# endoli/fiksi

Measured on AMD Instinct MI355X. Metric: Gauss-Newton iters/sec + converged systems/sec, 100k×32-constraint f64 batch, higher is better.
Workload: dtype f64

## Files before the change

fiksi_amd/csrc/fx_grouped.hip:

```cpp
#include <hip/hip_runtime.h>
#include <stdint.h>
#include <algorithm>
#include <cstdio>
#include <cstdlib>
#include <utility>

#include "fx_device.h"
#include "fx_expr.h"
#include "fx_grouped_rows.h"
#include "fx_wave.h"

#ifndef FX_GROUPED_LADDER
#define FX_GROUPED_LADDER 1
#endif

namespace fx {

struct GroupLayout {
    uint32_t vt, mr;
    uint32_t off_xs, off_a, off_rhs, off_g, off_r, off_p, off_gvar, off_rtag, off_vout, off_pw, off_pe;
    uint32_t off_colof, off_gcol, off_fidx;
    uint32_t pw_cap, pe_cap;
    uint32_t stride;
    uint32_t tab_bytes, off_qx;
// ... 626 lines not shown
                            const int tag = (int)(b.expr_tag[e0 + i] & 0x7F);
                            const ushort4 f4 = reinterpret_cast<const ushort4*>(b.expr_idx)[e0 + i];
                            uint16_t ff[4] = {f4.x, f4.y, f4.z, f4.w};
                            uint32_t vars8[8] = {0, 0, 0, 0, 0, 0, 0, 0};
                            const int k = expand_vars(tag, ff, vars8);
                            double prm_e = b.expr_param[e0 + i];
                            if ((prm.mode & 1u) && (tag == FX_TAG_PPD || tag == FX_TAG_PLD)) prm_e = scale_recip * prm_e;
                            rtag[pos] = (uint8_t)tag;
                            P[pos] = (T)prm_e;
#pragma unroll
                            for (int e = 0; e < 8; ++e) {
                                gvar[pos * 8 + e] = (uint16_t)vars8[e];
                                gcol[pos * 8 + e] = (e < k) ? (int8_t)colof[vars8[e]] : (int8_t)-1;
                            }
                        }
                    }
                }
                if (!UNITS && !reuse) {
                    nfree = 0;
                    bool any_var = false;
                    for_vars([&](uint32_t i, double v, uint32_t info) {
                        const bool member = i < nvt && (info & VAR_COMP_MASK) == c;
                        const bool in = member && !(info & VAR_FIXED_BIT);
                        const uint32_t m = gballot(in);
                        const uint32_t pos = nfree + (uint32_t)__popc(m & below);
                        if (i < nvt) colof[i] = in ? (int16_t)pos : (int16_t)-1;
                        if (in && pos < (uint32_t)N) fidx[pos] = (uint16_t)i;
                        if (i < (uint32_t)(RS * PF)) {
                            const int cc = in ? (int)pos : -1;
                            if (i < (uint32_t)RS) c_col[0] = cc; else if (i < 2u * RS) c_col[1] = cc; else c_col[2] = cc;
                        }
                        if (in && (prm.mode & 2u)) {
                            uint32_t st = lcg_jump(rng, 2u * pos);
                            st = st * 1664525u + 1013904223u;
                            const double f1 = (1.0 / 4294967295.0) * (double)st;
                            st = st * 1664525u + 1013904223u;
                            const double f2 = (1.0 / 4294967295.0) * (double)st;
                            double x = (prm.mode & 1u) ? v * scale_recip : v;
                            x += x * (1.0 / 8196.0) * f1 + (1.0 / 65568.0) * f2;
                            XS[i] = (T)x;
                        }
                        nfree += (uint32_t)__popc(m);
                        any_var = any_var || gballot(member) != 0u;
                    });
                    if (!any_var) {
                        c += 1;
                    } else {
                        have_comp = true;
                        rows_listed = true;
                        built = true;
                        built_cls = cls;
                        if (prm.mode & 2u) rng = lcg_jump(rng, 2u * nfree);
                        group_sync();
#pragma unroll
                        for (int q = 0; q < NC; ++q) {
                            const uint32_t j = (uint32_t)(hl + RS * q);
                            my_vi[q] = (j < nfree) ? (uint32_t)fidx[j] : 0u;
                        }
                        m_rows = 0;
                        for_exprs([&](uint32_t i, int tag, double prm_e, uint32_t comp, ushort4 f4) {
                            const bool in = (i < net) && (comp == c);
                            const uint32_t mk = gballot(in);
                            const uint32_t pos = m_rows + (uint32_t)__popc(mk & below);
                            if (i < (uint32_t)(RS * PF)) {
                                const int rr = in ? (int)pos : -1;
                                if (i < (uint32_t)RS) c_row[0] = rr; else if (i < 2u * RS) c_row[1] = rr; else c_row[2] = rr;
                            }
                            if (in) {
                                uint16_t ff[4] = {f4.x, f4.y, f4.z, f4.w};
                                uint32_t vars8[8] = {0, 0, 0, 0, 0, 0, 0, 0};
                                const int k = expand_vars(tag, ff, vars8);
                                if ((prm.mode & 1u) && (tag == FX_TAG_PPD || tag == FX_TAG_PLD)) prm_e = scale_recip * prm_e;
                                rtag[pos] = (uint8_t)tag;
                                P[pos] = (T)prm_e;
#pragma unroll
                                for (int e = 0; e < 8; ++e) {
                                    gvar[pos * 8 + e] = (uint16_t)vars8[e];
                                    gcol[pos * 8 + e] = (e < k) ? (int8_t)colof[vars8[e]] : (int8_t)-1;
                                }
                            }
                            m_rows += (uint32_t)__popc(mk);
                        });
                    }
                }
                if (rows_listed) {
                    group_sync();
#pragma unroll
                    for (int q = 0; q < NC; ++q) {
                        xstart[q] = ((uint32_t)(hl + RS * q) < nfree) ? XS[my_vi[q]] : T(0);
                        xc[q] = xstart[q];
                    }
                    n_pw = 0;
                    n_pe = 0;
                    for (uint32_t at = 0; !QRG && at < m_rows; at += RS) {
                        const uint32_t row = at + (uint32_t)hl;
                        uint32_t mask = 0;
                        uint64_t cols = 0;
                        if (row < m_rows) {
#pragma unroll
                            for (int e = 0; e < 8; ++e) {
                                const int cc = gcol[row * 8 + e];
                                mask |= (cc >= 0) ? (1u << e) : 0u;
                                cols |= (uint64_t)(uint8_t)cc << (8 * e);
                            }
                        }
                        const uint32_t kf = (uint32_t)__popc(mask);
                        uint32_t np = kf * (kf + 1u) / 2u;
                        for (uint32_t m1 = mask; m1; m1 &= m1 - 1u) {
                            const uint32_t a = (uint32_t)__ffs(m1) - 1u;
                            for (uint32_t m2 = m1 & (m1 - 1u); m2; m2 &= m2 - 1u) {
                                const uint32_t bb = (uint32_t)__ffs(m2) - 1u;
                                np += (((cols >> (8u * a)) ^ (cols >> (8u * bb))) & 0xFFu) == 0u;
                            }
                        }
                        uint32_t inc2 = np, inc1 = kf;
#pragma unroll
                        for (int off = 1; off < RS; off <<= 1) {
                            const uint32_t t2 = (uint32_t)__shfl_up((int)inc2, off, RS), t1 = (uint32_t)__shfl_up((int)inc1, off, RS);
                            if (hl >= off) {
                                inc2 += t2;
                                inc1 += t1;
                            }
                        }
                        uint32_t at2 = n_pw + inc2 - np, at1 = n_pe + inc1 - kf;
                        if (at2 + np <= L.pw_cap && at1 + kf <= L.pe_cap) {
                            for (uint32_t m1 = mask; m1; m1 &= m1 - 1u) {
                                const uint32_t a = (uint32_t)__ffs(m1) - 1u;
                                const uint32_t ca = (uint32_t)(cols >> (8u * a)) & 0xFFu;
                                PE[at1++] = (uint16_t)((row << (3 + CB)) | (a << CB) | ca);
                                for (uint32_t m2 = m1; m2; m2 &= m2 - 1u) {
                                    const uint32_t bb = (uint32_t)__ffs(m2) - 1u;
                                    const uint32_t cb = (uint32_t)(cols >> (8u * bb)) & 0xFFu;
                                    const uint32_t hi = ca > cb ? ca : cb, lo = ca > cb ? cb : ca;
                                    const uint32_t w = (row << 19) | (a << 16) | (bb << 13) | tri_at(hi, lo);
                                    PW[at2++] = w;
                                    if (a != bb && ca == cb) PW[at2++] = w;
                                }
                            }
                        }
                        n_pw += (uint32_t)__shfl((int)inc2, RS - 1, RS);
                        n_pe += (uint32_t)__shfl((int)inc1, RS - 1, RS);
                    }
                    group_sync();
                    if constexpr (PWR > 0) {
#pragma unroll
                        for (int u = 0; u < PWR; ++u) {
                            const uint32_t t = (uint32_t)(u * RS + hl);
                            pw_reg[u] = (t < n_pw && t < L.pw_cap) ? PW[t] : 0xFFFFFFFFu;
                        }
#pragma unroll
                        for (int u = 0; u < PER; ++u) {
                            const uint32_t t = (uint32_t)(u * RS + hl);
                            pe_reg[u] = (t < n_pe && t < L.pe_cap) ? (uint32_t)PE[t] : 0xFFFFFFFFu;
                        }
                    }
                }
                if (have_comp) {
                    stamp(GH_SETUP);
                    lambda = o.lambda0;
                    accepted = 0;
                    trials = 0;
                    outer = 0;
                    exit_code = FX_EXIT_MAX_OUTER;
                    fresh = true;
                    phase = GP_RUN;
                    if (n_pw > L.pw_cap || n_pe > L.pe_cap) {
                        sse = sse_start = T(0);
                        exit_code = FX_EXIT_NAN;
                        phase = GP_FINISH;
                    }
                }
            }
        }

        if constexpr (LADDER) {
            if (prm.ladder) {
                const unsigned long long bcand = __ballot(phase == GP_RUN && !fresh && lad_rank == 0);
                const unsigned long long bidle = __ballot(phase == GP_EXIT);
                if (bcand != 0ull && bidle != 0ull) {
                    uint32_t wid = 0, mem = 0, newlead = 0xFFFFu, newrank = 0;
#pragma unroll
                    for (int r = 0; r < 4; ++r) {
                        wid |= ((uint32_t)__builtin_amdgcn_readlane(lad_width, RS * r) & 15u) << (4 * r);
                        mem |= ((uint32_t)__builtin_amdgcn_readlane((int)lad_members, RS * r) & 255u) << (8 * r);
                    }
                    bool anyjoin = false;
#pragma unroll
                    for (int r = 0; r < 4; ++r) {
                        if (!((bidle >> (RS * r)) & 1ull)) continue;
                        uint32_t best = 15u, bw = 4u;
#pragma unroll
                        for (int l = 0; l < 4; ++l) {
                            const uint32_t w = (wid >> (4 * l)) & 15u;
                            if (((bcand >> (RS * l)) & 1ull) && w < bw) {
                                best = (uint32_t)l;
                                bw = w;
                            }
                        }
                        if (best != 15u) {
                            newlead = (newlead & ~(15u << (4 * r))) | (best << (4 * r));
                            newrank |= bw << (4 * r);
                            const uint32_t at = 8u * best + 2u * bw;
                            mem = (mem & ~(3u << at)) | ((uint32_t)r << at);
                            wid += 1u << (4u * best);
                            anyjoin = true;
                        }
                    }
                    if (anyjoin) {
                        const uint32_t nl = (newlead >> (4 * myrow)) & 15u;
                        const bool joining = nl != 15u;
                        const int grp = joining ? (int)nl : lad_lead;
                        const int srcl = grp * RS + hl;
                        auto cp = [&](auto& v) {
                            const auto t = lane_get(v, srcl);
                            if (joining) v = t;
                        };
                        cp(nfree); cp(m_rows); cp(n_pw); cp(n_pe); cp(trials); cp(accepted); cp(outer); cp(exit_code);
                        cp(sse); cp(lambda);
#pragma unroll
                        for (int q = 0; q < NC; ++q) {
                            cp(my_vi[q]); cp(xc[q]); cp(diag[q]); cp(rhs_l[q]);
                        }
                        if constexpr (PWR > 0) {
#pragma unroll
                            for (int u = 0; u < PWR; ++u) cp(pw_reg[u]);
#pragma unroll
                            for (int u = 0; u < PER; ++u) cp(pe_reg[u]);
                        }
                        lad_width = (int)((wid >> (4 * grp)) & 15u);
                        lad_members = (mem >> (8 * grp)) & 255u;
                        if (joining) {
                            lad_lead = (int)nl;
                            lad_rank = (int)((newrank >> (4 * myrow)) & 15u);
                            built = false;
                            using V = typename Vec16<T>::type;
                            const V* lb = reinterpret_cast<const V*>(rows0 + (uint32_t)nl * L.stride);
                            V* mine = reinterpret_cast<V*>(base);
                            for (uint32_t i = hl; i < L.stride / 16u; i += RS) mine[i] = lb[i];
                            fresh = false;
                            phase = GP_RUN;
                        }
                        group_sync();
                    }
                }
            }
        }

        int kmax;
        {
            const int km = (phase == GP_RUN && !fresh) ? (int)nfree : 0;
            const int k0 = __builtin_amdgcn_readlane(km, 0), k1 = __builtin_amdgcn_readlane(km, 16);
            const int k2 = __builtin_amdgcn_readlane(km, 32), k3 = __builtin_amdgcn_readlane(km, 48);
            kmax = max(max(k0, k1), max(k2, k3));
        }
        if (phase == GP_RUN) {
            stamp(GH_TAIL);
            int code = LC_FRESH;
            bool go = true;
            T delta[NC];
#pragma unroll
            for (int q = 0; q < NC; ++q) delta[q] = T(0);
            if (!fresh) {
                code = LC_REJECT;
                double lam_k = lambda;
                if constexpr (LADDER) {
                    if (lad_rank > 0)
                        for (int k = 0; k < lad_rank; ++k) lam_k *= o.reject_factor;
                }
                if (trials + (uint32_t)lad_rank >= o.max_trials) {
                    code = LC_CAP;
                    go = false;
                }
                if constexpr (QRG) {
                    if (go && !qr_step(lam_k, delta)) {
                        code = LC_SINGULAR;
                        go = false;
                    }
                }
                if (!QRG && go) {
                    int hv = hl;
                    asm volatile("" : "+v"(hv));
#pragma unroll
                    for (int q = 0; q < NC; ++q) At[tri_at((uint32_t)(hv + RS * q), (uint32_t)(hv + RS * q))] = diag[q] + (T)lam_k;
                    group_sync();
                    T a[NC][N];
#pragma unroll
                    for (int q = 0; q < NC; ++q) {
                        const int j = hv + RS * q;
                        const T* own = At + (uint32_t)(j * (j + 1) / 2);
                        const T* col = At + (uint32_t)j;
#pragma unroll
                        for (int i = 0; i < N; ++i) {
                            const int ti = i * (i + 1) / 2;
                            if (i <= RS * q) a[q][i] = own[i];
                            else if (i >= RS * (q + 1)) a[q][i] = col[ti];
                            else a[q][i] = ((hv >= i - RS * q) ? own : col + (ti - i))[i];
                        }
                    }
                    T invd[NC];
#pragma unroll
                    for (int q = 0; q < NC; ++q) invd[q] = T(1);
                    bool bad = false;
                    T acc[NC];
                    RBlock<NC, T, 0, UNITS>::template factor<false>(a, invd, acc, bad, hl, kmax);
                    stamp(GH_FACTOR);
                    if (bad) {
                        code = LC_SINGULAR;
                        go = false;
                    } else {
                        T invd2[NC];
#pragma unroll
                        for (int q = 0; q < NC; ++q) {
                            acc[q] = rhs_l[q];
                            invd2[q] = invd[q] * invd[q];
                        }
                        RBlock<NC, T, 0, UNITS>::forward(a, invd, acc, hl, kmax);
                        RBlock<NC, T, N / 8 - 1, UNITS>::backward(a, invd2, acc, hl, kmax);
#pragma unroll
                        for (int q = 0; q < NC; ++q) delta[q] = ((uint32_t)(hl + RS * q) < nfree) ? acc[q] * invd2[q] : T(0);
                    }
                }
                if (go) {
                    T dn2;
                    if constexpr (QRG) {
                        double acc = 0.0;
#pragma unroll
                        for (int q = 0; q < NC; ++q)
                            if ((uint32_t)(RS * q) < nfree) seq_add(acc, (double)delta[q] * (double)delta[q]);
                        dn2 = (T)acc;
                    } else {
                        dn2 = row_sum(delta[0] * delta[0]);
                        if constexpr (NC >= 2) dn2 = dn2 + row_sum(delta[1] * delta[1]);
                        if constexpr (NC >= 3) dn2 = dn2 + row_sum(delta[2] * delta[2]);
                    }
                    if (!(dn2 == dn2)) {
                        code = LC_NAN;
                        go = false;
                    } else if (dn2 < (T)o.step_tol) {
                        code = LC_STEP;
                        go = false;
                    }
                    stamp(GH_SOLVE);
                }
                if (go) {
#pragma unroll
                    for (int q = 0; q < NC; ++q)
                        if ((uint32_t)(hl + RS * q) < nfree) XS[my_vi[q]] = xc[q] + delta[q];
                    group_sync();
                }
            }
            T sse_t = T(0);
            if (go) {
                if constexpr (QRG) {
                    if (fresh) sse_t = eval_rows(std::true_type{});
                    else sse_t = eval_rows(std::false_type{});
                } else {
                    sse_t = eval_rows(std::true_type{});
                }
                stamp(GH_EVAL);
                if (!fresh) {
                    if (sse_t < sse) {
                        code = LC_ACCEPT;
                    } else {
                        double lam_k = lambda * o.reject_factor;
                        if constexpr (LADDER) {
                            if (lad_rank > 0)
                                for (int k = 0; k < lad_rank; ++k) lam_k *= o.reject_factor;
                        }
                        if (!(sse_t == sse_t) && !(lam_k < 1.0e300)) {
                            code = LC_REJ_NAN;
                        } else if (sizeof(T) == 4 && sse_t - sse <= (T)o.ftol * sse) {
                            code = LC_REJ_FTOL;
                        }
                    }
                }
            }
            int kw = (code != LC_REJECT) ? 0 : 1;
            int code_w = code;
            T sse_w = sse_t;
            T delta_w[NC];
#pragma unroll
            for (int q = 0; q < NC; ++q) delta_w[q] = delta[q];
            win_row = myrow;
            if constexpr (LADDER) {
                if (__ballot(lad_width > 1) != 0ull) {
                    int ck[4];
#pragma unroll
                    for (int k = 0; k < 4; ++k) ck[k] = lane_get(code, (int)((lad_members >> (2 * k)) & 3u) * RS + hl);
                    kw = lad_width;
                    code_w = LC_REJECT;
#pragma unroll
                    for (int k = 3; k >= 0; --k) {
                        if (k < lad_width && ck[k] != LC_REJECT) {
                            kw = k;
                            code_w = ck[k];
                        }
                    }
                    const int wrow = (int)((lad_members >> (2 * (kw < lad_width ? kw : 0))) & 3u);
                    const int wl = wrow * RS + hl;
                    sse_w = lane_get(sse_t, wl);
#pragma unroll
                    for (int q = 0; q < NC; ++q) delta_w[q] = lane_get(delta[q], wl);
                    win_row = wrow;
                }
            }
            bool assemble = false, fin = false;
            if (fresh) {
                sse = sse_t;
                sse_start = sse_t;
                assemble = true;
            } else {
                if (kw > 0) {
                    lambda *= o.reject_factor;
                    if constexpr (LADDER)
                        for (int k = 1; k < kw; ++k) lambda *= o.reject_factor;
                }
                if (kw == lad_width) {
                    trials += (uint32_t)kw;
                } else {
                    trials += (uint32_t)kw + (code_w != LC_CAP ? 1u : 0u);
                    if (code_w == LC_CAP) {
                        exit_code = FX_EXIT_TRIAL_CAP;
                        fin = true;
                    } else if (code_w == LC_SINGULAR) {
                        lambda *= o.singular_factor;
                    } else if (code_w == LC_NAN) {
                        exit_code = FX_EXIT_NAN;
                        fin = true;
                    } else if (code_w == LC_STEP) {
                        exit_code = FX_EXIT_STEP;
                        fin = true;
                    } else if (code_w == LC_ACCEPT) {
                        lambda *= o.accept_factor;
                        if (lambda < o.lambda_min) lambda = o.lambda_min;
#pragma unroll
                        for (int q = 0; q < NC; ++q)
                            if ((uint32_t)(hl + RS * q) < nfree) xc[q] = xc[q] + delta_w[q];
                        accepted += 1;
                        const T rel = (sse - sse_w) / sse;
                        sse = sse_w;
                        if (rel <= (T)o.ftol) {
                            exit_code = FX_EXIT_FTOL;
                            fin = true;
                        } else {
                            assemble = true;
                            outer += 1;
                        }
                    } else {
                        lambda *= o.reject_factor;
                        exit_code = (code_w == LC_REJ_NAN) ? FX_EXIT_NAN : FX_EXIT_FTOL;
                        fin = true;
                    }
                }
            }
            if (assemble) {
                if constexpr (QRG) {
                    if (!fresh) {
#pragma unroll
                        for (int q = 0; q < NC; ++q)
                            if ((uint32_t)(hl + RS * q) < nfree) XS[my_vi[q]] = xc[q];
                        group_sync();
                        (void)eval_rows(std::true_type{});
                    }
                } else if constexpr (LADDER) {
                    if (win_row != myrow) {
                        using V = typename Vec16<T>::type;
                        const unsigned char* wb = rows0 + (uint32_t)win_row * L.stride;
                        const V* gs = reinterpret_cast<const V*>(wb + L.off_g);
                        V* gd = reinterpret_cast<V*>(G);
                        const uint32_t ng = m_rows * 8u / (uint32_t)Vec16<T>::n;
                        for (uint32_t i = hl; i < ng; i += RS) gd[i] = gs[i];
                        const T* rs = reinterpret_cast<const T*>(wb + L.off_r);
                        for (uint32_t i = hl; i < m_rows; i += RS) R[i] = rs[i];
                        group_sync();
                    }
                }
                if constexpr (!QRG) form_normal();
                stamp(GH_FORM);
                if (fresh && (!(sse == sse) || !(sse < Lim<T>::huge()))) {
                    exit_code = FX_EXIT_NAN;
                    fin = true;
                } else if (outer >= o.max_outer) {
                    fin = true;
                } else if (sse < (T)o.sse_tol) {
                    exit_code = FX_EXIT_SSE;
                    fin = true;
                }
            }
            fresh = false;
            if (fin) {
                phase = GP_FINISH;
                if constexpr (LADDER) {
                    if (lad_rank > 0) {
                        phase = GP_EXIT;
                    }
                    lad_rank = 0;
                    lad_width = 1;
                    lad_lead = myrow;
                    lad_members = (uint32_t)myrow * 0x55u;
                }
            }
        }

        bool finish_now = phase == GP_FINISH;
        if (prm.hold_passes) {
            const int n_done = __popcll(__ballot(phase == GP_FINISH)) / RS;
            const bool any_running = __ballot(phase == GP_RUN) != 0ull;
            if (phase == GP_FINISH) {
                if (n_done >= 2 || !any_running || held >= prm.hold_passes) {
                    held = 0;
                } else {
                    held += 1;
                    finish_now = false;
                }
            }
        }
        if (finish_now) {
#pragma unroll
            for (int q = 0; q < NC; ++q) {
                if ((uint32_t)(hl + RS * q) < nfree) {
                    const double x = (double)xc[q];
                    const double xo = (prm.mode & 1u) ? scale * x : x;
                    b.vars[v0 + my_vi[q]] = xo;
                    VOUT[my_vi[q]] = xo;
                    XS[my_vi[q]] = (UNITS && !(unit_flags & UNIT_RESTORE)) ? xc[q] : xstart[q];
                }
            }
            group_sync();
            tot_accept += accepted;
            tot_trials += trials;
            last_exit = exit_code;
            tot_sse0 += (double)sse_start;
            tot_sse += (double)sse;
            if (!UNITS) comps_done += 1;
            c += 1;
            phase = GP_COMP;
            stamp(GH_TAIL);
        }

        if (phase == GP_COMP && c >= ncomp) {
                double part[4] = {0.0, 0.0, 0.0, 0.0};
                for_exprs([&](uint32_t i, int tag, double param, uint32_t, ushort4 f4) {
                    if (i < net) {
                        uint16_t ff[4] = {f4.x, f4.y, f4.z, f4.w};
                        uint32_t vars8[8] = {0, 0, 0, 0, 0, 0, 0, 0};
                        expand_vars(tag, ff, vars8);
                        double v[8], g[8];
#pragma unroll
                        for (int e = 0; e < 8; ++e) v[e] = VOUT[vars8[e]];
                        const double r = eval_expression<double, false, QRG>(tag, v, param, g);
                        const double r2 = r * r;
                        const uint32_t blk = (i >> 4) & 3u;
#pragma unroll
                        for (int q = 0; q < 4; ++q) part[q] += (blk == (uint32_t)q) ? r2 : 0.0;
                    }
                });
                const double sse_u = block_sum4(part);
                if (hl == 0) {
                    fx_result res;
                    res.accepted = tot_accept;
                    res.trials = tot_trials;
                    res.exit = last_exit;
                    res.ncomp = comps_done;
                    res.scale = scale;
                    res.sse0 = tot_sse0;
                    res.sse = tot_sse;
                    res.sse_unscaled = sse_u;
                    b.results[s] = res;
                }
                group_sync();
                phase = GP_NEXT;
                stamp(GH_SETUP);
        }

        if (__ballot(phase != GP_EXIT || (LADDER && prm.ladder && !qdone)) == 0ull) break;
    }
    if (PROF) {
        stamp(GH_TAIL);
        if (lane == 0 && prm.prof) {
            for (int i = 0; i < GH_COUNT; ++i) atomicAdd(&prm.prof[i], ph[i]);
        }
    }
}

template <int NC, typename T, bool PROF, bool UNITS>
__global__ __launch_bounds__(64) __attribute__((amdgpu_waves_per_eu(1, 1))) void lm_solve_grouped_kernel_w1(
    DeviceBatch b, LmParams prm, GroupLayout L, uint32_t* __restrict__ next_system) {
    extern __shared__ __align__(16) unsigned char smem[];
    grouped_body<NC, T, PROF, UNITS>(b, prm, L, next_system, smem);
}
__global__ __launch_bounds__(64) __attribute__((amdgpu_waves_per_eu(1, 1))) void lm_solve_grouped_qr_kernel(
    DeviceBatch b, LmParams prm, GroupLayout L, uint32_t* __restrict__ next_system) {
    extern __shared__ __align__(16) unsigned char smem[];
    grouped_body<2, double, false, false, true>(b, prm, L, next_system, smem);
}
template <int NC, typename T, bool PROF, bool UNITS>
__global__ __launch_bounds__(64) __attribute__((amdgpu_waves_per_eu(2))) void lm_solve_grouped_kernel_w2(
    DeviceBatch b, LmParams prm, GroupLayout L, uint32_t* __restrict__ next_system) {
    extern __shared__ __align__(16) unsigned char smem[];
    grouped_body<NC, T, PROF, UNITS>(b, prm, L, next_system, smem);
}

template <int NC, typename T, bool PROF = false, bool UNITS = false>
static hipError_t launch_grouped_t(const DeviceBatch& b, const LmParams& p, uint32_t* counter, hipStream_t stream) {
    const uint32_t rows = UNITS ? b.max_unit_rows : b.max_rows;
    const uint32_t pairs = UNITS ? (b.max_unit_rows * 64u < b.max_pairs_tri ? b.max_unit_rows * 64u : b.max_pairs_tri) : b.max_pairs_tri;
    const uint32_t ents = UNITS ? (b.max_unit_rows * 8u < b.max_ents ? b.max_unit_rows * 8u : b.max_ents) : b.max_ents;
// ... 156 lines not shown
```

fiksi_amd/csrc/fx_grouped_rows.h:

```cpp
#pragma once
#include <hip/hip_runtime.h>
#include <stdint.h>
#include <utility>

#include "fx_device.h"
#include "fx_expr.h"
#include "fx_wave.h"

namespace fx {

constexpr int RS = 16;

template <int K>
__device__ __forceinline__ double rbcast(double v) {
    return __longlong_as_double(__builtin_amdgcn_mov_dpp(__double_as_longlong(v), 0x150 + K, 0xF, 0xF, false));
}
template <int K>
__device__ __forceinline__ float rbcast(float v) {
    return __int_as_float(__builtin_amdgcn_mov_dpp(__float_as_int(v), 0x150 + K, 0xF, 0xF, false));
}
template <int K>
__device__ __forceinline__ void fnma_rbcast(double& acc, double m, double w) {
    asm volatile("v_fmac_f64_dpp %0, -%1, %2 row_newbcast:%3 row_mask:0xf bank_mask:0xf" : "+v"(acc) : "v"(m), "v"(w), "n"(K));
}
template <int K>
__device__ __forceinline__ void fnma_rbcast(float& acc, float m, float w) {
    asm volatile("v_fmac_f32_dpp %0, -%1, %2 row_newbcast:%3 row_mask:0xf bank_mask:0xf" : "+v"(acc) : "v"(m), "v"(w), "n"(K));
}
__device__ __forceinline__ void dpp_settle(double& v) { asm volatile("s_nop 1" : "+v"(v)); }
__device__ __forceinline__ void dpp_settle(float& v) { asm volatile("s_nop 1" : "+v"(v)); }
template <int K>
__device__ __forceinline__ void fnma_rbcast_self(double& acc, double w) {
    asm volatile("v_fmac_f64_dpp %0, -%0, %1 row_newbcast:%2 row_mask:0xf bank_mask:0xf" : "+v"(acc) : "v"(w), "n"(K));
}
template <int K>
__device__ __forceinline__ void fnma_rbcast_self(float& acc, float w) {
    asm volatile("v_fmac_f32_dpp %0, -%0, %1 row_newbcast:%2 row_mask:0xf bank_mask:0xf" : "+v"(acc) : "v"(w), "n"(K));
}
template <typename T>
__device__ __forceinline__ T row_sum(T v) {
    v += dpp_move<0xB1>(v);
    v += dpp_move<0x4E>(v);
    v += dpp_move<0x141>(v);
    v += dpp_move<0x140>(v);
    return v;
}
template <typename T>
__device__ __forceinline__ T block_sum4(const T (&acc)[4]) {
    return (row_sum(acc[0]) + row_sum(acc[1])) + (row_sum(acc[2]) + row_sum(acc[3]));
}
template <int... K>
__device__ __forceinline__ void seq_add_impl(double& sum, double t, std::integer_sequence<int, K...>) {
    ((sum += rbcast<K>(t)), ...);
}
__device__ __forceinline__ void seq_add(double& sum, double t) { seq_add_impl(sum, t, std::make_integer_sequence<int, RS>{}); }

template <int NC, typename T, int K, bool BOUNDED>
struct RStep {
    static constexpr int N = RS * NC;
    static constexpr int KA = K / RS, KL = K % RS;
    template <bool FWD>
    static __device__ __forceinline__ void factor(T (&a)[NC][N], T (&invd)[NC], T (&acc)[NC], bool& bad, int hl, int kmax) {
        {
        const T piv = rbcast<KL>(a[KA][K]);
        bad = bad || !(piv > T(0)) || !(piv < Lim<T>::huge());
        const T rs = rsqrt_refined(piv);
        const T ip = rs * rs;
        T mul[NC];
#pragma unroll
        for (int q = 0; q < NC; ++q) {
            mul[q] = T(0);
            if (q < KA) continue;
            const T ljk = a[q][K] * rs;
            const bool above = (q > KA) || (hl > KL);
            mul[q] = above ? a[q][K] * ip : T(0);
            if (above || hl == KL) a[q][K] = ljk;
            if (q == KA && hl == KL) invd[q] = rs;
        }
        if constexpr (NC <= 2) {
#pragma unroll
            for (int i = K + 1; i < N; ++i) {
#pragma unroll
                for (int q = NC - 1; q >= KA; --q) {
                    if (q == KA && KL == RS - 1) continue;
                    if (q == KA) fnma_rbcast_self<KL>(a[q][i], mul[q]);
                    else fnma_rbcast<KL>(a[q][i], a[KA][i], mul[q]);
                }
            }
            if constexpr (FWD) forward_dpp(a, rs, acc, hl);
            asm volatile("s_nop 1");
        } else {
#pragma unroll
            for (int i = K + 1; i < N; ++i) {
                const T aik = rbcast<KL>(a[KA][i]);
#pragma unroll
                for (int q = KA; q < NC; ++q) {
                    if (q == KA && KL == RS - 1) continue;
                    a[q][i] = fma(-aik, mul[q], a[q][i]);
                }
            }
            static_assert(!FWD, "the 48-column build substitutes in a pass of its own");
        }
        }
    }
    static __device__ __forceinline__ void forward_dpp(const T (&a)[NC][N], T invd_k, T (&acc)[NC], int hl) {
        T t = acc[KA] * invd_k;
        dpp_settle(t);
#pragma unroll
        for (int q = NC - 1; q >= KA; --q) {
            if (q == KA && KL == RS - 1) continue;
            const T w = (q > KA || hl > KL) ? a[q][K] : T(0);
            fnma_rbcast<KL>(acc[q], t, w);
        }
    }
    static __device__ __forceinline__ void forward(const T (&a)[NC][N], const T (&invd)[NC], T (&acc)[NC], int hl, int kmax) {
        {
        T t = acc[KA] * invd[KA];
        if constexpr (NC <= 2) {
            forward_dpp(a, invd[KA], acc, hl);
        } else {
            const T yk = rbcast<KL>(t);
#pragma unroll
            for (int q = KA; q < NC; ++q) {
                if (q == KA && KL == RS - 1) continue;
                if (q > KA || hl > KL) acc[q] = fma(-a[q][K], yk, acc[q]);
            }
        }
        }
    }
    static __device__ __forceinline__ void backward(const T (&a)[NC][N], const T (&invd2)[NC], T (&acc)[NC], int hl, int kmax) {
        {
        T t = acc[KA] * invd2[KA];
        if constexpr (NC <= 2) {
            dpp_settle(t);
#pragma unroll
            for (int q = 0; q <= KA; ++q) {
                if (q == KA && KL == 0) continue;
                const T w = (q < KA || hl < KL) ? a[q][K] : T(0);
                fnma_rbcast<KL>(acc[q], t, w);
            }
        } else {
            const T xi = rbcast<KL>(t);
#pragma unroll
            for (int q = 0; q <= KA; ++q) {
                if (q == KA && KL == 0) continue;
                if (q < KA || hl < KL) acc[q] = fma(-a[q][K], xi, acc[q]);
            }
        }
        }
    }
};

template <int NC, typename T, int KB, bool BOUNDED>
struct RBlock {
    static constexpr int N = RS * NC;
    template <bool FWD, int... I>
    static __device__ __forceinline__ void factor8(T (&a)[NC][N], T (&invd)[NC], T (&acc)[NC], bool& bad, int hl, int kmax, std::integer_sequence<int, I...>) {
        (RStep<NC, T, 8 * KB + I, BOUNDED>::template factor<FWD>(a, invd, acc, bad, hl, kmax), ...);
    }
    template <int... I>
    static __device__ __forceinline__ void forward8(const T (&a)[NC][N], const T (&invd)[NC], T (&acc)[NC], int hl, int kmax, std::integer_sequence<int, I...>) {
        (RStep<NC, T, 8 * KB + I, BOUNDED>::forward(a, invd, acc, hl, kmax), ...);
    }
    template <int... I>
    static __device__ __forceinline__ void backward8(const T (&a)[NC][N], const T (&invd2)[NC], T (&acc)[NC], int hl, int kmax, std::integer_sequence<int, I...>) {
        (RStep<NC, T, 8 * KB + 7 - I, BOUNDED>::backward(a, invd2, acc, hl, kmax), ...);
    }
    template <bool FWD>
    static __device__ __forceinline__ void factor(T (&a)[NC][N], T (&invd)[NC], T (&acc)[NC], bool& bad, int hl, int kmax) {
        if (!BOUNDED || 8 * KB < kmax) factor8<FWD>(a, invd, acc, bad, hl, kmax, std::make_integer_sequence<int, 8>{});
        if constexpr (8 * KB + 8 < N) RBlock<NC, T, KB + 1, BOUNDED>::template factor<FWD>(a, invd, acc, bad, hl, kmax);
    }
    static __device__ __forceinline__ void forward(const T (&a)[NC][N], const T (&invd)[NC], T (&acc)[NC], int hl, int kmax) {
        if (!BOUNDED || 8 * KB < kmax) forward8(a, invd, acc, hl, kmax, std::make_integer_sequence<int, 8>{});
        if constexpr (8 * KB + 8 < N) RBlock<NC, T, KB + 1, BOUNDED>::forward(a, invd, acc, hl, kmax);
    }
    static __device__ __forceinline__ void backward(const T (&a)[NC][N], const T (&invd2)[NC], T (&acc)[NC], int hl, int kmax) {
        if (!BOUNDED || 8 * KB < kmax) backward8(a, invd2, acc, hl, kmax, std::make_integer_sequence<int, 8>{});
        if constexpr (KB > 0) RBlock<NC, T, KB - 1, BOUNDED>::backward(a, invd2, acc, hl, kmax);
    }
};

__device__ __forceinline__ void group_sync() {
    __builtin_amdgcn_fence(__ATOMIC_RELEASE, "wavefront");
    __builtin_amdgcn_wave_barrier();
    __builtin_amdgcn_fence(__ATOMIC_ACQUIRE, "wavefront");
}

enum GroupPhase : int { GP_NEXT = 0, GP_COMP = 1, GP_RUN = 2, GP_FINISH = 3, GP_EXIT = 4 };

enum LadderCode : int {
    LC_REJECT = 0,
    LC_SINGULAR = 1,
    LC_NAN = 2,
    LC_STEP = 3,
    LC_ACCEPT = 4,
    LC_REJ_NAN = 5,
    LC_REJ_FTOL = 6,
    LC_CAP = 7,
    LC_FRESH = 8
};

__device__ __forceinline__ int lane_get(int v, int src_lane) { return __builtin_amdgcn_ds_bpermute(src_lane << 2, v); }
__device__ __forceinline__ uint32_t lane_get(uint32_t v, int src_lane) { return (uint32_t)__builtin_amdgcn_ds_bpermute(src_lane << 2, (int)v); }
__device__ __forceinline__ float lane_get(float v, int src_lane) { return __int_as_float(__builtin_amdgcn_ds_bpermute(src_lane << 2, __float_as_int(v))); }
__device__ __forceinline__ double lane_get(double v, int src_lane) {
    const int lo = __builtin_amdgcn_ds_bpermute(src_lane << 2, __double2loint(v));
    const int hi = __builtin_amdgcn_ds_bpermute(src_lane << 2, __double2hiint(v));
    return __hiloint2double(hi, lo);
}

}
```

Baseline: 57.34 million.

## Software-pipeline Cholesky pivot prologue into previous step's row updates

```diff
diff --git a/fiksi_amd/csrc/fx_grouped.hip b/fiksi_amd/csrc/fx_grouped.hip
--- a/fiksi_amd/csrc/fx_grouped.hip
+++ b/fiksi_amd/csrc/fx_grouped.hip
@@ -952,7 +952,8 @@
                     for (int q = 0; q < NC; ++q) invd[q] = T(1);
                     bool bad = false;
                     T acc[NC];
-                    RBlock<NC, T, 0, UNITS>::template factor<false>(a, invd, acc, bad, hl, kmax);
+                    constexpr bool LOOK = !(NC == 2 && sizeof(T) == 4);
+                    RBlock<NC, T, 0, UNITS>::template factor<false, LOOK>(a, invd, acc, bad, hl, kmax);
                     stamp(GH_FACTOR);
                     if (bad) {
                         code = LC_SINGULAR;
diff --git a/fiksi_amd/csrc/fx_grouped_rows.h b/fiksi_amd/csrc/fx_grouped_rows.h
--- a/fiksi_amd/csrc/fx_grouped_rows.h
+++ b/fiksi_amd/csrc/fx_grouped_rows.h
@@ -29,6 +29,15 @@
 }
 __device__ __forceinline__ void dpp_settle(double& v) { asm volatile("s_nop 1" : "+v"(v)); }
 __device__ __forceinline__ void dpp_settle(float& v) { asm volatile("s_nop 1" : "+v"(v)); }
+__device__ __forceinline__ void pin(double& v) { asm volatile("" ::"v"(v)); }
+__device__ __forceinline__ void pin(float& v) { asm volatile("" ::"v"(v)); }
+template <int W, typename T>
+__device__ __forceinline__ void settle_after(T& v) {
+    if constexpr (W < 2) asm volatile("s_nop %1" : "+v"(v) : "n"(1 - W));
+    else asm volatile("" : "+v"(v));
+}
+__device__ __forceinline__ double rsq_seed(double p) { return __builtin_amdgcn_rsq(p); }
+__device__ __forceinline__ float rsq_seed(float p) { return __builtin_amdgcn_rsqf(p); }
 template <int K>
 __device__ __forceinline__ void fnma_rbcast_self(double& acc, double w) {
     asm volatile("v_fmac_f64_dpp %0, -%0, %1 row_newbcast:%2 row_mask:0xf bank_mask:0xf" : "+v"(acc) : "v"(w), "n"(K));
@@ -55,10 +64,125 @@
 }
 __device__ __forceinline__ void seq_add(double& sum, double t) { seq_add_impl(sum, t, std::make_integer_sequence<int, RS>{}); }
 
+template <int NC, typename T>
+struct RPro {
+    T p, y, m, h, e, ip, t;
+    T mul[NC];
+};
+
 template <int NC, typename T, int K, bool BOUNDED>
 struct RStep {
     static constexpr int N = RS * NC;
     static constexpr int KA = K / RS, KL = K % RS;
+
+    static constexpr int C = NC - KA - (KL == RS - 1 ? 1 : 0);
+    static constexpr int R = N - K - 2;
+    static constexpr int NEWTON = sizeof(T) == 8 ? 2 : 1;
+    static constexpr int NL = 2 + 3 * NEWTON + 2;
+    static constexpr int fc(bool fwd) { return fwd ? C : 0; }
+    static constexpr int p0(bool fwd) {
+        for (int j = 0; j <= R; ++j)
+            if (fc(fwd) + j * C >= 2) return j;
+        return R;
+    }
+    static constexpr int lpos(int l, bool fwd) { return p0(fwd) + l * (R - p0(fwd) + 1) / NL; }
+    static constexpr int after(int l, bool fwd) { return (R - lpos(l, fwd)) * C; }
+
+    template <int L, bool FWD, int W0>
+    static __device__ __forceinline__ void pro(RPro<NC, T>& s, T (&a)[NC][N], T (&invd)[NC], const T (&acc)[NC], bool& bad, int hl) {
+        if constexpr (L == 0) {
+            settle_after<W0>(a[KA][K]);
+            s.p = rbcast<KL>(a[KA][K]);
+            bad = bad || !(s.p > T(0)) || !(s.p < Lim<T>::huge());
+            pin(s.p);
+        } else if constexpr (L == 1) {
+            s.y = rsq_seed(s.p);
+            pin(s.y);
+        } else if constexpr (L < 2 + 3 * NEWTON) {
+            constexpr int r = (L - 2) % 3;
+            if constexpr (r == 0) {
+                s.m = -s.p * s.y;
+                s.h = T(0.5) * s.y;
+                pin(s.m);
+                pin(s.h);
+            } else if constexpr (r == 1) {
+                s.e = fma(s.m, s.y, T(1));
+                pin(s.e);
+            } else {
+                s.y = fma(s.h, s.e, s.y);
+                pin(s.y);
+            }
+        } else if constexpr (L == NL - 2) {
+            s.ip = s.y * s.y;
+            pin(s.ip);
+            if constexpr (FWD) {
+                s.t = acc[KA] * s.y;
+                pin(s.t);
+            }
+        } else {
+            const T rs = s.y;
+#pragma unroll
+            for (int q = 0; q < NC; ++q) {
+                s.mul[q] = T(0);
+                if (q < KA) continue;
+                const T ljk = a[q][K] * rs;
+                const bool above = (q > KA) || (hl > KL);
+                s.mul[q] = above ? a[q][K] * s.ip : T(0);
+                if (above || hl == KL) a[q][K] = ljk;
+                if (q == KA && hl == KL) invd[q] = rs;
+                pin(s.mul[q]);
+            }
+        }
+    }
+    template <bool FWD, int W0, int... L>
+    static __device__ __forceinline__ void pro_all(RPro<NC, T>& s, T (&a)[NC][N], T (&invd)[NC], const T (&acc)[NC], bool& bad, int hl, std::integer_sequence<int, L...>) {
+        (pro<L, FWD, L == 0 ? W0 : 2>(s, a, invd, acc, bad, hl), ...);
+    }
+    template <bool FWD, int W0>
+    static __device__ __forceinline__ void prologue(RPro<NC, T>& s, T (&a)[NC][N], T (&invd)[NC], const T (&acc)[NC], bool& bad, int hl) {
+        pro_all<FWD, W0>(s, a, invd, acc, bad, hl, std::make_integer_sequence<int, NL>{});
+    }
+    template <int I>
+    static __device__ __forceinline__ void row(T (&a)[NC][N], const T (&mul)[NC]) {
+#pragma unroll
+        for (int q = NC - 1; q >= KA; --q) {
+            if (q == KA && KL == RS - 1) continue;
+            if (q == KA) fnma_rbcast_self<KL>(a[q][I], mul[q]);
+            else fnma_rbcast<KL>(a[q][I], a[KA][I], mul[q]);
+        }
+    }
+    using Next = RStep<NC, T, K + 1, BOUNDED>;
+    template <bool FWD, bool LOOK, int J, int... L>
+    static __device__ __forceinline__ void at(T (&a)[NC][N], T (&invd)[NC], const T (&acc)[NC], bool& bad, int hl, const T (&mul)[NC], RPro<NC, T>& nx, std::integer_sequence<int, L...>) {
+        if constexpr (J > 0) row<K + 1 + J>(a, mul);
+        if constexpr (LOOK)
+            ((lpos(L, FWD) == J ? Next::template pro<L, FWD, fc(FWD) + J * C>(nx, a, invd, acc, bad, hl) : void()), ...);
+    }
+    template <bool FWD, bool LOOK, int... J>
+    static __device__ __forceinline__ void rows(T (&a)[NC][N], T (&invd)[NC], const T (&acc)[NC], bool& bad, int hl, const T (&mul)[NC], RPro<NC, T>& nx, std::integer_sequence<int, J...>) {
+        (at<FWD, LOOK, J>(a, invd, acc, bad, hl, mul, nx, std::make_integer_sequence<int, NL>{}), ...);
+    }
+    template <bool FWD, bool LOOK, int TG>
+    static __device__ __forceinline__ void update(T (&a)[NC][N], T (&invd)[NC], T (&acc)[NC], bool& bad, int hl, RPro<NC, T>& s, RPro<NC, T>& nx) {
+        if constexpr (K + 1 < N) row<K + 1>(a, s.mul);
+        if constexpr (FWD && C > 0) {
+            settle_after<TG + (K + 1 < N ? C : 0)>(s.t);
+            forward_fmacs(a, s.t, acc, hl);
+        }
+        if constexpr (K + 1 < N) rows<FWD, LOOK>(a, invd, acc, bad, hl, s.mul, nx, std::make_integer_sequence<int, R + 1>{});
+        if constexpr (K + 2 < N && Next::C > 0) {
+            constexpr int w = (R - 1) * C;
+            if constexpr (w < 2) asm volatile("s_nop %0" ::"n"(1 - w));
+        }
+    }
+    template <bool FWD, int KE, int TG>
+    static __device__ __forceinline__ void run(T (&a)[NC][N], T (&invd)[NC], T (&acc)[NC], bool& bad, int hl, RPro<NC, T>& s) {
+        RPro<NC, T> nx;
+        constexpr bool look = K + 1 < KE;
+        update<FWD, look, TG>(a, invd, acc, bad, hl, s, nx);
+        if constexpr (look) Next::template run<FWD, KE, after(NL - 2, FWD)>(a, invd, acc, bad, hl, nx);
+    }
+
     template <bool FWD>
     static __device__ __forceinline__ void factor(T (&a)[NC][N], T (&invd)[NC], T (&acc)[NC], bool& bad, int hl, int kmax) {
         {
@@ -103,15 +227,18 @@
         }
         }
     }
-    static __device__ __forceinline__ void forward_dpp(const T (&a)[NC][N], T invd_k, T (&acc)[NC], int hl) {
-        T t = acc[KA] * invd_k;
-        dpp_settle(t);
+    static __device__ __forceinline__ void forward_fmacs(const T (&a)[NC][N], T t, T (&acc)[NC], int hl) {
 #pragma unroll
         for (int q = NC - 1; q >= KA; --q) {
             if (q == KA && KL == RS - 1) continue;
             const T w = (q > KA || hl > KL) ? a[q][K] : T(0);
             fnma_rbcast<KL>(acc[q], t, w);
         }
+    }
+    static __device__ __forceinline__ void forward_dpp(const T (&a)[NC][N], T invd_k, T (&acc)[NC], int hl) {
+        T t = acc[KA] * invd_k;
+        dpp_settle(t);
+        forward_fmacs(a, t, acc, hl);
     }
     static __device__ __forceinline__ void forward(const T (&a)[NC][N], const T (&invd)[NC], T (&acc)[NC], int hl, int kmax) {
         {
@@ -166,10 +293,29 @@
     static __device__ __forceinline__ void backward8(const T (&a)[NC][N], const T (&invd2)[NC], T (&acc)[NC], int hl, int kmax, std::integer_sequence<int, I...>) {
         (RStep<NC, T, 8 * KB + 7 - I, BOUNDED>::backward(a, invd2, acc, hl, kmax), ...);
     }
-    template <bool FWD>
+    template <bool FWD, bool LOOK = true>
     static __device__ __forceinline__ void factor(T (&a)[NC][N], T (&invd)[NC], T (&acc)[NC], bool& bad, int hl, int kmax) {
-        if (!BOUNDED || 8 * KB < kmax) factor8<FWD>(a, invd, acc, bad, hl, kmax, std::make_integer_sequence<int, 8>{});
-        if constexpr (8 * KB + 8 < N) RBlock<NC, T, KB + 1, BOUNDED>::template factor<FWD>(a, invd, acc, bad, hl, kmax);
+        if constexpr (NC <= 2 && LOOK) {
+            using First = RStep<NC, T, 8 * KB, BOUNDED>;
+            if constexpr (!BOUNDED) {
+                static_assert(KB == 0, "the unbounded factorization is one piece");
+                RPro<NC, T> s;
+                First::template prologue<FWD, 2>(s, a, invd, acc, bad, hl);
+                First::template run<FWD, N, 0>(a, invd, acc, bad, hl, s);
+            } else {
+                using Prev = RStep<NC, T, (KB > 0 ? 8 * KB - 1 : 0), BOUNDED>;
+                constexpr int w0 = KB > 0 ? Prev::fc(FWD) + Prev::R * Prev::C : 2;
+                if (8 * KB < kmax) {
+                    RPro<NC, T> s;
+                    First::template prologue<FWD, w0>(s, a, invd, acc, bad, hl);
+                    First::template run<FWD, 8 * KB + 8, 0>(a, invd, acc, bad, hl, s);
+                }
+            }
+        } else {
+            if (!BOUNDED || 8 * KB < kmax) factor8<FWD>(a, invd, acc, bad, hl, kmax, std::make_integer_sequence<int, 8>{});
+        }
+        if constexpr ((!(NC <= 2 && LOOK) || BOUNDED) && 8 * KB + 8 < N)
+            RBlock<NC, T, KB + 1, BOUNDED>::template factor<FWD, LOOK>(a, invd, acc, bad, hl, kmax);
     }
     static __device__ __forceinline__ void forward(const T (&a)[NC][N], const T (&invd)[NC], T (&acc)[NC], int hl, int kmax) {
         if (!BOUNDED || 8 * KB < kmax) forward8(a, invd, acc, hl, kmax, std::make_integer_sequence<int, 8>{});
```

Result: faster. 58.03 million, median of 6 (+1.2%).
